# mit-han-lab/pvcnn

Hardware: AMD Instinct MI355X
Metric: point-clouds/sec fwd+bwd, PVCNN S3DIS N=4096 R=32 (higher is better)
Workload: dtype f32 (fp32 tensors, fp32 accumulate; Conv3d fwd / bwd-data / bwd-weight and the large SharedMLP fwd / bwd-data / bwd-weight products as power-of-two scaled fp16 hi+lo splits, 3 partial products on fp16 MFMA, max rel err vs fp64 1e-6 <= the fp32-MFMA kernels'; PVCNN_CONV_MATH=fp32 PVCNN_PW_MATH=fp32 s; 1 GPU; PVCNN (1xC) S3DIS fwd+bwd+Adam, B=16/GPU N=4096 R=32/16 fp32; global_batch=16, points=4096, parallelism=dp1, gradient_bytes=10289972, step_mode=graph, rccl_ranks=0, gradient_buckets=2

## Files before the change

include/pvcnn_hip.h:

```cpp
#ifndef PVCNN_HIP_H_
#define PVCNN_HIP_H_

#include <stddef.h>
#include <stdint.h>

#ifdef __cplusplus
extern "C" {
#endif

#if defined(__GNUC__)
#define PVCNN_API __attribute__((visibility("default")))
#else
#define PVCNN_API
#endif

#define PVCNN_ABI_VERSION 17
#define PVCNN_OK 0
#define PVCNN_ERR_INVALID_ARGUMENT (-1)

PVCNN_API int pvcnn_version(void);
PVCNN_API const char *pvcnn_last_error_string(void);

PVCNN_API int pvcnn_voxel_coords(const float *coords, int B, int N, int R, int normalize, float eps, float *norm_coords,
                       int32_t *vox_coords, void *stream);

PVCNN_API int pvcnn_voxel_coords_tail(const float *coords, long coords_batch_stride, const float *mean, const float *radius,
                            int B, int N, int R, float eps, float *norm_coords, int32_t *vox_coords, void *stream);

PVCNN_API size_t pvcnn_avg_voxelize_fwd_workspace_bytes(int B, int C, int N, int R);
PVCNN_API int pvcnn_avg_voxelize_fwd(const float *feat, const int32_t *coords, int B, int C, int N, int R,
                           float *out, int32_t *ind, int32_t *cnt, void *workspace,
                           size_t workspace_bytes, void *stream);
PVCNN_API int pvcnn_avg_voxelize_bwd(const float *grad_y, const int32_t *ind, const int32_t *cnt, int B,
                           int C, int N, int S, float *grad_x, void *stream);

PVCNN_API int pvcnn_trilinear_devox_fwd(const float *coords, const float *feat, int B, int C, int N, int R,
                              int is_training, int32_t *inds, float *wgts, float *outs,
                              void *stream);
PVCNN_API size_t pvcnn_trilinear_devox_bwd_workspace_bytes(int B, int C, int N, int R);
PVCNN_API int pvcnn_trilinear_devox_bwd(const float *grad_y, const int32_t *inds, const float *wgts, int B,
                              int C, int N, int R, float *grad_x, void *workspace,
                              size_t workspace_bytes, void *stream);

PVCNN_API size_t pvcnn_avg_voxelize_plan_bytes(int B, int N, int R);
PVCNN_API size_t pvcnn_avg_voxelize_plan_scratch_bytes(int B, int N, int R);
PVCNN_API int pvcnn_avg_voxelize_plan(const int32_t *coords, int B, int N, int R, int32_t *ind, int32_t *cnt, void *plan,
                            size_t plan_bytes, void *scratch, size_t scratch_bytes, void *stream);
PVCNN_API size_t pvcnn_pvconv_plans_scratch_bytes(int B, int N, int R);
PVCNN_API int pvcnn_pvconv_plans(const int32_t *vox_coords, const float *norm_coords, int B, int N, int R, int32_t *ind, int32_t *cnt,
                                 void *vox_plan, size_t vox_plan_bytes, void *devox_bwd_plan, size_t devox_bwd_plan_bytes,
                                 void *scratch, size_t scratch_bytes, void *stream);
PVCNN_API int pvcnn_avg_voxelize_apply(const float *feat, const void *plan, size_t plan_bytes, int B, int C, int N, int R,
                             float *out, void *stream);
PVCNN_API size_t pvcnn_trilinear_devox_bwd_plan_bytes(int B, int N, int R);
PVCNN_API size_t pvcnn_trilinear_devox_bwd_plan_scratch_bytes(int B, int N, int R);
PVCNN_API int pvcnn_trilinear_devox_bwd_plan(const int32_t *inds, const float *wgts, int B, int N, int R, void *plan,
                                   size_t plan_bytes, void *scratch, size_t scratch_bytes, void *stream);
PVCNN_API int pvcnn_trilinear_devox_bwd_apply(const float *grad_y, long grad_y_batch_stride, const void *plan, size_t plan_bytes,
                                    int B, int C, int N, int R, float *grad_x, void *stream);

PVCNN_API int pvcnn_ball_query(const float *centers, const float *points, int B, int N, int M, float radius,
                     int U, int32_t *out, void *stream);

PVCNN_API int pvcnn_grouping_fwd(const float *features, const int32_t *indices, int B, int C, int N, int M,
                       int U, float *out, void *stream);
PVCNN_API size_t pvcnn_grouping_bwd_workspace_bytes(int B, int C, int N, int M, int U);
PVCNN_API int pvcnn_grouping_bwd(const float *grad_y, const int32_t *indices, int B, int C, int N, int M,
// ... 387 lines not shown
```

pvcnn_amd/_lib.py:

```python
import ctypes
import functools
import os

import torch

_CSRC = os.path.join(os.path.dirname(os.path.abspath(__file__)), 'csrc')
LIB_PATH = os.path.join(_CSRC, 'libpvcnn_hip.so')
ABI_VERSION = 17

_vp, _i, _f, _sz, _l = ctypes.c_void_p, ctypes.c_int, ctypes.c_float, ctypes.c_size_t, ctypes.c_long
_ll = ctypes.c_longlong
_d = ctypes.c_double

SIGNATURES = {
    'pvcnn_version': (_i, []),
    'pvcnn_last_error_string': (ctypes.c_char_p, []),
    'pvcnn_voxel_coords': (_i, [_vp, _i, _i, _i, _i, _f, _vp, _vp, _vp]),
    'pvcnn_voxel_coords_tail': (_i, [_vp, ctypes.c_long, _vp, _vp, _i, _i, _i, _f, _vp, _vp, _vp]),
    'pvcnn_avg_voxelize_fwd_workspace_bytes': (_sz, [_i, _i, _i, _i]),
    'pvcnn_avg_voxelize_fwd': (_i, [_vp, _vp, _i, _i, _i, _i, _vp, _vp, _vp, _vp, _sz, _vp]),
    'pvcnn_avg_voxelize_bwd': (_i, [_vp, _vp, _vp, _i, _i, _i, _i, _vp, _vp]),
    'pvcnn_trilinear_devox_fwd': (_i, [_vp, _vp, _i, _i, _i, _i, _i, _vp, _vp, _vp, _vp]),
    'pvcnn_trilinear_devox_bwd_workspace_bytes': (_sz, [_i, _i, _i, _i]),
    'pvcnn_trilinear_devox_bwd': (_i, [_vp, _vp, _vp, _i, _i, _i, _i, _vp, _vp, _sz, _vp]),
    'pvcnn_avg_voxelize_plan_bytes': (_sz, [_i, _i, _i]),
    'pvcnn_avg_voxelize_plan_scratch_bytes': (_sz, [_i, _i, _i]),
    'pvcnn_avg_voxelize_plan': (_i, [_vp, _i, _i, _i, _vp, _vp, _vp, _sz, _vp, _sz, _vp]),
    'pvcnn_avg_voxelize_apply': (_i, [_vp, _vp, _sz, _i, _i, _i, _i, _vp, _vp]),
    'pvcnn_pvconv_plans_scratch_bytes': (_sz, [_i, _i, _i]),
    'pvcnn_pvconv_plans': (_i, [_vp, _vp, _i, _i, _i, _vp, _vp, _vp, _sz, _vp, _sz, _vp, _sz, _vp]),
    'pvcnn_trilinear_devox_bwd_plan_bytes': (_sz, [_i, _i, _i]),
    'pvcnn_trilinear_devox_bwd_plan_scratch_bytes': (_sz, [_i, _i, _i]),
    'pvcnn_trilinear_devox_bwd_plan': (_i, [_vp, _vp, _i, _i, _i, _vp, _sz, _vp, _sz, _vp]),
    'pvcnn_trilinear_devox_bwd_apply': (_i, [_vp, ctypes.c_long, _vp, _sz, _i, _i, _i, _i, _vp, _vp]),
    'pvcnn_ball_query': (_i, [_vp, _vp, _i, _i, _i, _f, _i, _vp, _vp]),
    'pvcnn_grouping_fwd': (_i, [_vp, _vp, _i, _i, _i, _i, _i, _vp, _vp]),
    'pvcnn_grouping_bwd_workspace_bytes': (_sz, [_i, _i, _i, _i, _i]),
    'pvcnn_grouping_bwd': (_i, [_vp, _vp, _i, _i, _i, _i, _i, _vp, _vp, _sz, _vp]),
    'pvcnn_gather_fwd': (_i, [_vp, _vp, _i, _i, _i, _i, _vp, _vp]),
    'pvcnn_gather_bwd_workspace_bytes': (_sz, [_i, _i, _i, _i]),
    'pvcnn_gather_bwd': (_i, [_vp, _vp, _i, _i, _i, _i, _vp, _vp, _sz, _vp]),
    'pvcnn_fps': (_i, [_vp, _i, _i, _i, _vp, _vp, _vp]),
    'pvcnn_mask_select': (_i, [_vp, _i, _i, _i, _vp, _vp, _vp, _vp, _vp]),
    'pvcnn_three_nn_interp_fwd': (_i, [_vp, _vp, _vp, _i, _i, _i, _i, _vp, _vp, _vp, _vp]),
    'pvcnn_three_nn_interp_bwd_workspace_bytes': (_sz, [_i, _i, _i, _i]),
    'pvcnn_three_nn_interp_bwd': (_i, [_vp, _vp, _vp, _i, _i, _i, _i, _vp, _vp, _sz, _vp]),
    'pvcnn_conv3d_weight_transform': (_i, [_vp, _i, _i, _i, _vp, _vp]),
    'pvcnn_conv3d_fwd': (_i, [_vp, _vp, _vp, _i, _i, _i, _i, _vp, _vp]),
    'pvcnn_conv3d_bwd_weight_workspace_bytes': (_sz, [_i, _i, _i, _i]),
    'pvcnn_conv3d_bwd_weight': (_i, [_vp, _vp, _i, _i, _i, _i, _vp, _vp, _vp, _sz, _vp]),
    'pvcnn_conv3d_weight_split_bytes': (_sz, [_i, _i, _i, _i]),
    'pvcnn_conv3d_weight_split': (_i, [_vp, _i, _i, _i, _i, _vp, _vp]),
    'pvcnn_conv3d_weight_split_pair': (_i, [_vp, _i, _i, _vp, _vp, _vp]),
    'pvcnn_conv3d_fwd_split_stats_parts': (_sz, [_i, _i, _i, _i]),
# ... 180 lines not shown
```

pvcnn_amd/csrc/slab.h:

```cpp
#pragma once
#include <algorithm>
#include <stdlib.h>

#include "common.h"

namespace pvcnn {

template <int NC>
struct Taps {
  int32_t idx[NC];
  float w[NC];
};

__device__ __forceinline__ float4 ld4(const float *p) { return *reinterpret_cast<const float4 *>(p); }
__device__ __forceinline__ int4 ld4(const int32_t *p) { return *reinterpret_cast<const int4 *>(p); }
__device__ __forceinline__ void st4(float *p, float a, float b, float c, float d) {
  *reinterpret_cast<float4 *>(p) = make_float4(a, b, c, d);
}
__device__ __forceinline__ void st4(int32_t *p, int a, int b, int c, int d) {
  *reinterpret_cast<int4 *>(p) = make_int4(a, b, c, d);
}

template <int NC, bool MAY_SKIP, bool PAD = false>
__device__ __forceinline__ float combine(const Taps<NC> &t, const float *row, int pshift = 0) {
// ... 191 lines not shown
};
struct XfBnAct {
  static constexpr bool kIdentity = false;
  static constexpr int kRaw = 5;
  const float *gamma, *beta, *mean, *rstd;
  float slope;
  const float *se = nullptr;
  __device__ __forceinline__ XfBnAct at(int b_times_C) const {
    XfBnAct x = *this;
    if (x.se) x.se += b_times_C;
    return x;
  }
  __device__ __forceinline__ void params(int c, float &scale, float &shift) const {
    scale = (gamma ? gamma[c] : 1.0f) * rstd[c];
    shift = (beta ? beta[c] : 0.0f) - mean[c] * scale;
  }
  __device__ __forceinline__ float mul(int c) const { return se ? se[c] : 1.0f; }
  __device__ __forceinline__ float apply(float v, float scale, float shift, float m = 1.0f) const {
    v = fmaf(v, scale, shift);
    v = v > 0.f ? v : v * slope;
    return se ? v * m : v;
  }
  __device__ __forceinline__ void fetch(int c, float (&raw)[5]) const {
    raw[0] = gamma ? gamma[c] : 1.0f; raw[1] = rstd[c]; raw[2] = beta ? beta[c] : 0.0f; raw[3] = mean[c]; raw[4] = mul(c);
  }
  __device__ __forceinline__ void combine(const float (&raw)[5], float &scale, float &shift) const {
    scale = raw[0] * raw[1];
    shift = raw[2] - raw[3] * scale;
  }
};

struct AddPlain {
  static constexpr bool kPlain = true;
};
struct AddBnAct {
  static constexpr bool kPlain = false;
  const float *gamma, *beta, *mean, *rstd;
  float slope;
  __device__ __forceinline__ void params(int c, float &scale, float &shift) const {
    scale = (gamma ? gamma[c] : 1.0f) * rstd[c];
    shift = (beta ? beta[c] : 0.0f) - mean[c] * scale;
  }
  __device__ __forceinline__ float apply(float a, float scale, float shift) const {
    const float v = fmaf(a, scale, shift);
    return v > 0.f ? v : v * slope;
  }
};

template <int THREADS, class XF>
__device__ __forceinline__ void slab_copy_row_xf(float *dst, const float *src, int len, const XF &xf, int c) {
  float scale, shift;
  xf.params(c, scale, shift);
  const float m = xf.mul(c);
  if (((reinterpret_cast<uintptr_t>(src) | reinterpret_cast<uintptr_t>(dst)) & 15) == 0 && (len & 3) == 0) {
    constexpr int kB = 8;
    const int nq = len >> 2;
    const float4 *s4 = reinterpret_cast<const float4 *>(src);
    float4 *d4 = reinterpret_cast<float4 *>(dst);
    for (int q0 = threadIdx.x; q0 < nq; q0 += THREADS * kB) {
      float4 v[kB];
#pragma unroll
      for (int u = 0; u < kB; ++u) v[u] = s4[min(q0 + u * THREADS, nq - 1)];
#pragma unroll
      for (int u = 0; u < kB; ++u)
        if (q0 + u * THREADS < nq)
          d4[q0 + u * THREADS] = make_float4(xf.apply(v[u].x, scale, shift, m), xf.apply(v[u].y, scale, shift, m),
                                             xf.apply(v[u].z, scale, shift, m), xf.apply(v[u].w, scale, shift, m));
    }
  } else {
    for (int i = threadIdx.x; i < len; i += THREADS) dst[i] = xf.apply(src[i], scale, shift, m);
  }
}

template <int THREADS, class XF>
__device__ __forceinline__ void slab_copy_row_padded(float *dst, const float *src, int len, int pshift, const XF &xf, int c) {
  float scale = 1.0f, shift = 0.0f;
  [[maybe_unused]] float m = 1.0f;
  if constexpr (!XF::kIdentity) { xf.params(c, scale, shift); m = xf.mul(c); }
  auto f = [&](float v) {
// ... 33 lines not shown

template <class P, int VEC, int THREADS, bool RESIDENT, class XF, bool PAD, class AX = AddPlain>
__global__ __launch_bounds__(THREADS) void gather_lds_kernel(P p, XF xf, const float *__restrict__ src,
                                                             float *__restrict__ dst, int C, int L,
                                                             int J, int G, int SEQ, int pshift,
                                                             const float *__restrict__ addend = nullptr, AX ax = AX{}) {
  extern __shared__ __attribute__((aligned(16))) float lds[];
  constexpr int NC = P::NC;
  const int b = blockIdx.y;
  const XF xfb = xf.at(b * C);
  const bool side = (blockIdx.x == 0);
  constexpr bool resident = RESIDENT;
  const int jf = threadIdx.x * VEC;
  typename P::Packed pk[VEC];
  if (resident && jf < J) {
    if constexpr (VEC == 4) p.pack4(b, jf, pk); else p.pack1(b, jf, pk[0]);
    if (side) {
      Taps<NC> t[VEC];
#pragma unroll
      for (int v = 0; v < VEC; ++v) p.unpack(pk[v], t[v]);
      if constexpr (VEC == 4) p.post4(b, jf, t); else p.post1(b, jf, t[0]);
    }
  }
  for (int sq = 0; sq < SEQ; ++sq) {
    const int c0 = (blockIdx.x * SEQ + sq) * G;
    if (c0 >= C) break;
    const int g = min(G, C - c0);
    if (sq > 0) lds_barrier();
    const int Lp = PAD ? L + (L >> pshift) : L;
    slab_stage<THREADS, PAD>(lds, src + ((size_t)b * C + c0) * L, g, L, Lp, pshift, xfb, c0);
    __syncthreads();
    float *out = dst + ((size_t)b * C + c0) * J;
    const float *add = addend ? addend + ((size_t)b * C + c0) * J : nullptr;
    for (int j0 = jf; j0 < J; j0 += THREADS * VEC) {
      Taps<NC> t[VEC];
      if constexpr (resident) {
#pragma unroll
        for (int v = 0; v < VEC; ++v) p.unpack(pk[v], t[v]);
      } else if constexpr (VEC == 4) {
        p.load4(b, j0, t);
        if (side && sq == 0) p.post4(b, j0, t);
      } else {
        p.load1(b, j0, t[0]);
        if (side && sq == 0) p.post1(b, j0, t[0]);
      }
      for (int c = 0; c < g; ++c) {
        const float *row = lds + c * Lp;
        [[maybe_unused]] float ascale = 1.0f, ashift = 0.0f;
        if constexpr (!AX::kPlain) ax.params(c0 + c, ascale, ashift);
        if constexpr (VEC == 4) {
          const float r0 = combine<NC, P::kMaySkip, PAD>(t[0], row, pshift), r1 = combine<NC, P::kMaySkip, PAD>(t[1], row, pshift);
          float r2 = combine<NC, P::kMaySkip, PAD>(t[2], row, pshift), r3 = combine<NC, P::kMaySkip, PAD>(t[3], row, pshift);
          float q0 = r0, q1 = r1;
          if (add) {
            float4 a = ld4(add + (size_t)c * J + j0);
            if constexpr (!AX::kPlain)
              a = make_float4(ax.apply(a.x, ascale, ashift), ax.apply(a.y, ascale, ashift), ax.apply(a.z, ascale, ashift), ax.apply(a.w, ascale, ashift));
            q0 = q0 + a.x; q1 = q1 + a.y; r2 = r2 + a.z; r3 = r3 + a.w;
          }
          st4(out + (size_t)c * J + j0, q0, q1, r2, r3);
        } else {
          float r = combine<NC, P::kMaySkip, PAD>(t[0], row, pshift);
          if (add) {
            float a = add[(size_t)c * J + j0];
            if constexpr (!AX::kPlain) a = ax.apply(a, ascale, ashift);
            r = r + a;
          }
          out[(size_t)c * J + j0] = r;
        }
      }
    }
  }
}

template <class P, class XF, class AX = AddPlain>
__global__ __launch_bounds__(1024) void gather_lds_pipe_kernel(P p, XF xf, const float *__restrict__ src, float *__restrict__ dst,
                                                               int C, int L, int J, int SEQ, int pshift,
                                                               const float *__restrict__ addend = nullptr, AX ax = AX{}) {
  extern __shared__ __attribute__((aligned(16))) float lds[];
  constexpr int NC = P::NC, THREADS = 1024, kB = 8;
  const int b = blockIdx.y;
  const XF xfb = xf.at(b * C);
  const int jf = threadIdx.x * 4;
  const bool has = jf < J;
  const int nq = L >> 2;
  float4 v[kB];
  typedef unsigned int u32x4 __attribute__((ext_vector_type(4)));
  const int voff = (int)threadIdx.x * 16;
  auto row_descriptor = [&](const float *base, size_t off, int bytes) {
    const uintptr_t rowp = reinterpret_cast<uintptr_t>(base + off);
    const uint32_t lo = __builtin_amdgcn_readfirstlane((uint32_t)rowp), hi = __builtin_amdgcn_readfirstlane((uint32_t)(rowp >> 32));
    return __builtin_amdgcn_make_buffer_rsrc(reinterpret_cast<void *>(((uintptr_t)hi << 32) | lo),  0,
                                              __builtin_amdgcn_readfirstlane(bytes), 0x00020000);
  };
  auto load = [&](const __amdgpu_buffer_rsrc_t &rsrc, int u) {
    const u32x4 raw = __builtin_amdgcn_raw_buffer_load_b128(rsrc, voff, u * THREADS * 16, 0);
// ... 268 lines not shown

template <class K>
inline int enable_big_lds(K kernel, size_t bytes) {
  if (bytes > 64 * 1024)
    return (int)hipFuncSetAttribute(reinterpret_cast<const void *>(kernel),
                                    hipFuncAttributeMaxDynamicSharedMemorySize, (int)bytes);
  return 0;
}

template <class P, class XF = XfNone, class AX = AddPlain>
int launch_gather(const P &p, const float *src, float *dst, int B, int C, int L, int J, bool vec_ok,
                  hipStream_t s, const char *what, const XF &xf = XF{}, int pshift = 0, const float *addend = nullptr,
                  const AX &ax = AX{}) {
  if (B == 0 || C == 0 || J == 0) return 0;
  if (!AX::kPlain && !addend) {
    set_error("%s: an addend transform needs an addend", what);
    return PVCNN_ERR_INVALID_ARGUMENT;
  }
  if (pshift > 0 && (size_t)(L + (L >> pshift)) * sizeof(float) > (size_t)kLdsBytesPerCU) pshift = 0;
  SlabPlan pl = plan_slab(B, C, L, pshift);
  if constexpr (P::kGridRows) {
    if (switches().gather_pipe && pl.lds && pshift > 0 && vec_ok && J <= 1024 * 4 && J > 1024 && (L >> 2) == 1024 && aligned16(src) && C >= 4) {
      constexpr int GR = 2;
      const int slabs = ceil_div(C, GR);
      const int seq = (int)std::min<long>(8, std::max<long>(1, (long)B * slabs / kNumCU));
      const size_t bytes = (size_t)GR * (L + (L >> pshift)) * sizeof(float);
      auto k = gather_lds_pipe_rows_kernel<P, XF, GR, AX>;
      if (int e = enable_big_lds(k, bytes)) { set_error("%s: LDS attribute: %d", what, e); return e; }
      hipLaunchKernelGGL(k, dim3(ceil_div(slabs, seq), B), dim3(1024), bytes, s, p, xf, src, dst, C, L, J, seq, pshift, addend, ax);
      return check_launch(what);
    }
  }
  if (!pl.lds) {
    if (!XF::kIdentity || addend || !AX::kPlain) {
      set_error("%s: row does not fit LDS; the fused transform / addend needs the LDS path", what);
      return PVCNN_ERR_INVALID_ARGUMENT;
    } else if constexpr (XF::kIdentity) {
      const int CT = 16;
      hipLaunchKernelGGL((gather_direct_kernel<P>), dim3(ceil_div(J, 256), ceil_div(C, CT), B), dim3(256), 0, s,
                         p, src, dst, C, L, J, CT);
      return check_launch(what);
    }
  }
  const dim3 grid(ceil_div(ceil_div(C, pl.G), pl.seq), B);
  if constexpr (P::kGridRows) {
    if (switches().gather_pipe && pl.threads == 1024 && pl.G == 1 && pshift > 0 && vec_ok && J <= 1024 * 4 && (L & 3) == 0 && (L >> 2) <= 1024 * 8 &&
        aligned16(src) && (((size_t)L * sizeof(float)) & 15) == 0) {
      auto k = gather_lds_pipe_kernel<P, XF, AX>;
      if (int e = enable_big_lds(k, pl.bytes)) { set_error("%s: LDS attribute: %d", what, e); return e; }
      hipLaunchKernelGGL(k, grid, dim3(1024), pl.bytes, s, p, xf, src, dst, C, L, J, pl.seq, pshift, addend, ax);
      return check_launch(what);
    }
  }
#define PVCNN_LAUNCH_GATHER_P(VEC, T, PADV)                                                      \
  do {                                                                                           \
    auto k = (J <= T * VEC) ? gather_lds_kernel<P, VEC, T, true, XF, PADV, AX> : gather_lds_kernel<P, VEC, T, false, XF, PADV, AX>; \
    if (int e = enable_big_lds(k, pl.bytes)) { set_error("%s: LDS attribute: %d", what, e); return e; } \
    hipLaunchKernelGGL(k, grid, dim3(T), pl.bytes, s, p, xf, src, dst, C, L, J, pl.G, pl.seq, pshift, addend, ax); \
  } while (0)
#define PVCNN_LAUNCH_GATHER(VEC, T)                                                              \
  do {                                                                                           \
    if constexpr (P::kGridRows) { if (pshift > 0) PVCNN_LAUNCH_GATHER_P(VEC, T, true); else PVCNN_LAUNCH_GATHER_P(VEC, T, false); } \
    else PVCNN_LAUNCH_GATHER_P(VEC, T, false);                                                   \
  } while (0)
  if (pl.threads == 1024) { if (vec_ok) PVCNN_LAUNCH_GATHER(4, 1024); else PVCNN_LAUNCH_GATHER(1, 1024); }
  else                    { if (vec_ok) PVCNN_LAUNCH_GATHER(4, 256);  else PVCNN_LAUNCH_GATHER(1, 256); }
#undef PVCNN_LAUNCH_GATHER
// ... 19 lines not shown
```

pvcnn_amd/csrc/voxelize.hip:

```cpp
#include <algorithm>

#include "csr.h"

namespace pvcnn {

__global__ __launch_bounds__(256) void vox_stats_atomic_kernel(const int32_t *__restrict__ coords, int N,
                                                               int R, int S, int32_t *__restrict__ ind,
                                                               int32_t *__restrict__ cnt) {
  const int b = blockIdx.y, i = blockIdx.x * 256 + threadIdx.x;
  if (i >= N) return;
  const int32_t *co = coords + (size_t)b * 3 * N;
  int v = co[i] * R * R + co[i + N] * R + co[i + 2 * N];
  v = min(max(v, 0), S - 1);
  ind[(size_t)b * N + i] = v;
  atomicAdd(cnt + (size_t)b * S + v, 1);
}

__global__ __launch_bounds__(256) void vox_scatter_atomic_kernel(
    const float *__restrict__ feat, const int32_t *__restrict__ ind, const int32_t *__restrict__ cnt, int C,
    int N, int S, int CT, float *__restrict__ out) {
  const int b = blockIdx.z, i = blockIdx.x * 256 + threadIdx.x;
  if (i >= N) return;
  const int pos = ind[(size_t)b * N + i];
  const int cur = cnt[(size_t)b * S + pos];
// ... 147 lines not shown
  if (!csr_supported(S, N)) {
    PVCNN_HIP_TRY(hipMemsetAsync(cnt, 0, (size_t)B * S * 4, s));
    PVCNN_HIP_TRY(hipMemsetAsync(out, 0, (size_t)B * C * S * 4, s));
    if (N == 0) return 0;
    hipLaunchKernelGGL(vox_stats_atomic_kernel, dim3(ceil_div(N, 256), B), dim3(256), 0, s, coords, N, R, S, ind, cnt);
    if (int e = check_launch("vox_stats_atomic")) return e;
    if (C == 0) return 0;
    const int CT = 16;
    hipLaunchKernelGGL(vox_scatter_atomic_kernel, dim3(ceil_div(N, 256), ceil_div(C, CT), B), dim3(256), 0, s,
                       feat, ind, cnt, C, N, S, CT, out);
    return check_launch("vox_scatter_atomic");
  }

  VoxelEntries ep{coords, ind, N, R, S};
  return launch_csr_scatter(ep, feat, out, B, C, S, N, N, cnt, workspace, workspace_bytes, s,
                            "avg_voxelize_fwd");
}

extern "C" int pvcnn_avg_voxelize_bwd(const float *grad_y, const int32_t *ind, const int32_t *cnt, int B, int C,
                                      int N, int S, float *grad_x, void *stream) {
  PVCNN_REQUIRE(B >= 0 && C >= 0 && N >= 0 && S > 0, "negative size");
  if (B == 0 || C == 0 || N == 0) return 0;
  PVCNN_REQUIRE(grad_y && ind && cnt && grad_x, "null pointer");
  PVCNN_REQUIRE(B <= 65535, "batch > 65535");
  VoxelMean p{ind, cnt, N, S};
  const bool vec = (N % 4 == 0) && aligned16(ind) && aligned16(grad_x);
  int pshift = 0;
  for (int k = 2; k <= 10; ++k)
    if ((1L << (3 * k)) == (long)S) pshift = k;
  return launch_gather(p, grad_y, grad_x, B, C, S, N, vec, static_cast<hipStream_t>(stream),
                       "avg_voxelize_bwd", XfNone{}, pshift);
}

extern "C" size_t pvcnn_avg_voxelize_plan_bytes(int B, int N, int R) {
  if (B <= 0 || N < 0 || R <= 0) return 0;
  const long S = (long)R * R * R;
  if (S > 0x7fffffffL / 4 || !csr_supported((int)S, N)) return 0;
  return CsrPlan::bytes(B, (int)S, N);
}

extern "C" size_t pvcnn_avg_voxelize_plan_scratch_bytes(int B, int N, int R) {
  if (B <= 0 || N < 0 || R <= 0) return 0;
  return csr_prep_scratch_bytes(B, N);
}

extern "C" int pvcnn_avg_voxelize_plan(const int32_t *coords, int B, int N, int R, int32_t *ind, int32_t *cnt, void *plan,
                                       size_t plan_bytes, void *scratch, size_t scratch_bytes, void *stream) {
  PVCNN_REQUIRE(B >= 0 && N >= 0 && R > 0, "negative size");
  PVCNN_REQUIRE((long)R * R * R <= 0x7fffffffL / 4, "resolution too large");
  const int S = R * R * R;
  if (B == 0) return 0;
  PVCNN_REQUIRE(csr_supported(S, N), "grid too large for a plan: use pvcnn_avg_voxelize_fwd");
  PVCNN_REQUIRE(cnt && (ind || N == 0) && (coords || N == 0), "null pointer");
  PVCNN_REQUIRE(B <= 65535, "batch > 65535");
  VoxelEntries ep{coords, ind, N, R, S};
  return launch_csr_prep(ep, B, S, N, cnt, plan, plan_bytes, scratch, scratch_bytes, static_cast<hipStream_t>(stream),
                         "avg_voxelize_plan");
}

extern "C" size_t pvcnn_pvconv_plans_scratch_bytes(int B, int N, int R) {
  if (B <= 0 || N < 0 || R <= 0) return 0;
  return csr_prep_scratch_bytes(B, N) + csr_prep_scratch_bytes(B, 8L * N);
}

extern "C" int pvcnn_pvconv_plans(const int32_t *vox_coords, const float *norm_coords, int B, int N, int R, int32_t *ind, int32_t *cnt,
                                  void *vox_plan, size_t vox_plan_bytes, void *devox_bwd_plan, size_t devox_bwd_plan_bytes, void *scratch,
// ... 51 lines not shown
```

pvcnn_amd/modules/functional/_product.py:

```python
from typing import Callable, NamedTuple

from . import _cache, _gradslots
from ._align import aligned as _aligned


class Product(NamedTuple):
    kind: str
    c: str
    canon: Callable
    canon_w: Callable
    shaped: Callable
    out_shape: Callable
    wgrad_shape: Callable
    bias_dims: tuple
    amax_seg: Callable
    amax_tiles: Callable
    stats_parts: Callable
    wgrad_f16_ok: Callable
    amax: str
    weight_images: str
    product_split: str

    def entry(self, lib, name):
        return getattr(lib, f'pvcnn_{self.c}_{name}')

    def method(self, be, name):
        return getattr(be, f'{self.c}_{name}')


def _same(t, shape=None):
    return t


CONV = Product(
    kind='conv', c='conv3d',
    canon=_same, canon_w=_same, shaped=_same,
    out_shape=lambda b, c, r: (b, c, r, r, r), wgrad_shape=lambda co, ci: (co, ci, 3, 3, 3), bias_dims=(0, 2, 3, 4),
    amax_seg=lambda be, r: r, amax_tiles=lambda b, r, seg: b * r * r,
    stats_parts=lambda b, c, r, nsplit: (b, c, r, nsplit),
    wgrad_f16_ok=lambda be, x, w: True,
    amax='conv_amax', weight_images='conv_weight_images', product_split='conv3d_igemm_split')

PW = Product(
    kind='pw', c='pwconv',
    canon=lambda t: t.view(t.shape[0], t.shape[1], -1), canon_w=lambda w: w.view(w.shape[0], w.shape[1]),
    shaped=lambda t, shape: t.view(shape),
    out_shape=lambda b, c, n: (b, c, n), wgrad_shape=lambda co, ci: (co, ci), bias_dims=(0, 2),
    amax_seg=lambda be, n: be.PW_AMAX_SEG, amax_tiles=lambda b, n, seg: b * ((n + seg - 1) // seg),
    stats_parts=lambda b, c, n, nsplit: (b, n),
    wgrad_f16_ok=lambda be, x, w: x.shape[0] * x.shape[2] * w.shape[0] * w.shape[1] >= getattr(be, 'pw_wgrad_f16_min_macs', 0),
    amax='pw_amax', weight_images='pw_weight_images', product_split='pwconv_gemm_split')


def forward(p, be, ctx, given, weight, bias, want_stats, nsplit):
    x, w = p.canon(_aligned(given)), p.canon_w(weight.contiguous())
    ctx.save_for_backward(x, w)
    ctx.has_bias, ctx.x_shape, ctx.w_shape = bias is not None, given.shape, weight.shape
    ctx.bias_param = bias
    ctx.nsplit = int(nsplit)
    b = bias.contiguous() if bias is not None else None
    ctx.x_amax = None
    if ctx.nsplit in (1, 2):
        ctx.x_amax = _cache.amax_of(given, p.amax_seg(be, x.shape[2]))
        if ctx.x_amax is None and ctx.nsplit == 2:
            ctx.x_amax = getattr(be, p.amax)(x, want_global=False)
    kw = {'amax': ctx.x_amax} if ctx.nsplit == 2 else {}
    ctx.w_bwd_image = None
    if ctx.nsplit and hasattr(be, p.weight_images) and ctx.needs_input_grad[0]:
        w_image, ctx.w_bwd_image = getattr(be, p.weight_images)(w, ctx.nsplit)
        run = lambda **k: getattr(be, p.product_split)(x, w_image, b, w.shape[0], ctx.nsplit, amax=ctx.x_amax, **k)
    elif ctx.nsplit:
        run = lambda **k: p.method(be, 'forward_split')(x, w, b, ctx.nsplit, **kw, **k)
    else:
        run = lambda **k: p.method(be, 'forward')(x, w, b, **k)
    y_shape = (given.shape[0], w.shape[0], *given.shape[2:])
    if want_stats:
        y, part = run(want_stats=True)
        ctx.mark_non_differentiable(part)
        ctx.set_materialize_grads(False)
        return p.shaped(y, y_shape), part
    return p.shaped(run(), y_shape)


def backward(p, be, ctx, received):
    x, w = ctx.saved_tensors
    if received is None:
        return None, None, None, None, None
    grad_y = p.canon(_aligned(received))
    f16 = ctx.nsplit == 2
    wgrad_f16 = (ctx.nsplit in (1, 2) and ctx.needs_input_grad[1] and p.method(be, 'backward_weight_f16_serves')(x)
                 and p.wgrad_f16_ok(be, x, w))
    g_amax = None
    if (f16 and (ctx.needs_input_grad[0] or wgrad_f16)) or (ctx.nsplit == 1 and wgrad_f16):
        g_amax = _cache.amax_of(received, p.amax_seg(be, grad_y.shape[2]))
        if g_amax is None and f16:
            g_amax = getattr(be, p.amax)(grad_y, want_global=False)
    gx = None
    if ctx.needs_input_grad[0]:
        if ctx.nsplit and ctx.w_bwd_image is not None:
            rows = getattr(ctx, 'need_rows', None)
            gx = getattr(be, p.product_split)(grad_y, ctx.w_bwd_image, None, w.shape[1], ctx.nsplit, False, g_amax,
                                              **({'rows': rows} if rows is not None else {}))
        elif ctx.nsplit:
            gx = p.method(be, 'backward_data_split')(grad_y, w, ctx.nsplit, **({'amax': g_amax} if f16 else {}))
        else:
            gx = p.method(be, 'backward_data')(grad_y, w)
        gx = p.shaped(gx, ctx.x_shape)
    want_bias = ctx.has_bias and ctx.needs_input_grad[2]
    gw = gb = None
    if ctx.needs_input_grad[1]:
        dst = _gradslots.destinations(be, w, ctx.bias_param if want_bias else None)
        res = (p.method(be, 'backward_weight_f16')(x, grad_y, ctx.x_amax, g_amax, with_bias=want_bias, **dst) if wgrad_f16
               else p.method(be, 'backward_weight')(x, grad_y, with_bias=want_bias, **dst))
        gw, gb = res if want_bias else (res, None)
        gw = p.shaped(gw, ctx.w_shape)
    elif want_bias:
        gb = grad_y.sum(dim=p.bias_dims)
    return gx, gw, gb, None, None
```

pvcnn_amd/modules/functional/backend.py:

```python
import ctypes
import os

import torch

from ... import _lib
from . import _cache
from ._align import aligned as _aligned
from ._product import CONV, PW

__all__ = ['_backend']


def _dev(t, name):
    if not t.is_cuda:
        raise RuntimeError(f'{name} must be a CUDA (HIP) tensor -- the PVConv hot path has no CPU implementation')


def _f32(t, name):
    _dev(t, name)
    if not t.is_contiguous():
        raise RuntimeError(f'{name} must be a contiguous tensor')
    if t.dtype != torch.float32:
        raise RuntimeError(f'{name} must be a float tensor')

# ... 335 lines not shown
               'avg_voxelize: features (B,C,N), coords (B,3,N) expected')
        b, c, n = features.shape
        r = int(resolution)
        s3 = r * r * r
        dev = features.device
        if self.seam_plan_memo and self.lib.pvcnn_avg_voxelize_plan_bytes(b, n, r):
            key = ('seam voxelize plan', r)
            hit = _cache.memo(coords, key, lambda: self._stamped_voxel_plan(coords, r))
            if hit is not None and (hit[0].ind._version, hit[0].cnt._version) != hit[1]:
                _cache.forget(coords, key)
                hit = _cache.memo(coords, key, lambda: self._stamped_voxel_plan(coords, r))
            if hit is not None:
                return [self.avg_voxelize_apply(features, hit[0]), hit[0].ind, hit[0].cnt]
        out = torch.empty((b, c, s3), dtype=torch.float32, device=dev)
        ind = torch.empty((b, n), dtype=torch.int32, device=dev)
        cnt = torch.empty((b, s3), dtype=torch.int32, device=dev)
        ws = self._scratch(self.lib.pvcnn_avg_voxelize_fwd_workspace_bytes(b, c, n, r), dev)
        _run(self.lib.pvcnn_avg_voxelize_fwd, 'avg_voxelize_forward', features, features, coords, b, c, n, r, out, ind, cnt, ws, ws.numel())
        return [out, ind, cnt]

    def _stamped_voxel_plan(self, coords, r):
        vp = self.avg_voxelize_plan(coords, r)
        return None if vp is None else (vp, (vp.ind._version, vp.cnt._version))

    def avg_voxelize_backward(self, grad_y, indices, cnt):
        _f32(grad_y, 'grad_y'); _i32(indices, 'indices'); _i32(cnt, 'cnt')
        _shape(grad_y.dim() == 3 and indices.dim() == 2 and tuple(cnt.shape) == (grad_y.shape[0], grad_y.shape[2])
               and indices.shape[0] == grad_y.shape[0],
               'avg_voxelize backward: grad_y (B,C,S), indices (B,N), cnt (B,S) expected')
        b, c, s3 = grad_y.shape
        n = indices.shape[1]
        grad_x = torch.empty((b, c, n), dtype=torch.float32, device=grad_y.device)
        _run(self.lib.pvcnn_avg_voxelize_bwd, 'avg_voxelize_backward', grad_y, grad_y, indices, cnt, b, c, n, s3, grad_x)
        return grad_x

    has_scatter_plans = True

    class VoxelPlan:
        __slots__ = ('ind', 'cnt', 'plan', 'r', 'n', 'b')

    def _voxel_plan(self, b, n, r, nbytes, dev):
        vp = self.VoxelPlan()
        vp.r, vp.n, vp.b = r, n, b
        vp.ind = torch.empty((b, n), dtype=torch.int32, device=dev)
        vp.cnt = torch.empty((b, r * r * r), dtype=torch.int32, device=dev)
        vp.plan = torch.empty((nbytes,), dtype=torch.uint8, device=dev)
        return vp

    def avg_voxelize_plan(self, coords, resolution):
        _i32(coords, 'coords')
        _shape(coords.dim() == 3 and coords.shape[1] == 3, 'avg_voxelize: coords (B,3,N) expected')
        b, _, n = coords.shape
        r = int(resolution)
        nbytes = self.lib.pvcnn_avg_voxelize_plan_bytes(b, n, r)
        if nbytes == 0:
            return None
        vp = self._voxel_plan(b, n, r, nbytes, coords.device)
        scratch = self._scratch(self.lib.pvcnn_avg_voxelize_plan_scratch_bytes(b, n, r), coords.device)
        _run(self.lib.pvcnn_avg_voxelize_plan, 'avg_voxelize_plan', coords, coords, b, n, r, vp.ind, vp.cnt, vp.plan, vp.plan.numel(),
             scratch, scratch.numel())
        return vp

    has_conv_bwd_rows = True

    def voxel_need_rows(self, cnt, resolution):
        _i32(cnt, 'cnt')
# ... 1121 lines not shown
```

pvcnn_amd/modules/functional/voxelization.py:

```python
from torch.autograd import Function

from . import _cache
from ._autograd import native, amp_fwd, amp_bwd

__all__ = ['avg_voxelize']


class AvgVoxelization(Function):

    @staticmethod
    @amp_fwd
    def forward(ctx, features, coords, resolution):
        r = int(resolution)
        feats = features.contiguous()
        be = native()
        plan = None
        if feats.is_cuda and getattr(be, 'has_scatter_plans', False):
            plan = _cache.memo(coords, ('avg_voxelize_plan', r), lambda: be.avg_voxelize_plan(coords.int().contiguous(), r))
        if plan is not None:
            grid, point_voxel, voxel_count = be.avg_voxelize_apply(feats, plan), plan.ind, plan.cnt
        else:
            grid, point_voxel, voxel_count = be.avg_voxelize_forward(feats, coords.int().contiguous(), r)
        ctx.save_for_backward(point_voxel, voxel_count)
        return grid.view(feats.shape[0], feats.shape[1], r, r, r)

    @staticmethod
    @amp_bwd
    def backward(ctx, grad_grid):
        point_voxel, voxel_count = ctx.saved_tensors
        nb, nc = grad_grid.shape[0], grad_grid.shape[1]
        flat = grad_grid.contiguous().view(nb, nc, -1)
        return native().avg_voxelize_backward(flat, point_voxel, voxel_count), None, None


avg_voxelize = AvgVoxelization.apply
```

pvcnn_amd/modules/pvconv.py:

```python
import torch
import torch.nn as nn

from . import functional as F
from .functional._autograd import native
from .functional.bnact import (batch_norm_act_devoxelize, batch_norm_act_devoxelize_point_bn, batch_norm_act_se_devoxelize, fusable_tail,
                               point_bn_fusable, run_layers, _has_hooks)
from .functional.conv3d import conv_nsplit, voxel_conv3d
from .se import SE3d
from .shared_mlp import SharedMLP
from .voxelization import Voxelization

__all__ = ['PVConv']


class _VoxelConv3d(nn.Conv3d):

    def _fast(self, x):
        return (x.is_cuda and getattr(native(), 'has_conv3d', False) and self.kernel_size == (3, 3, 3)
                and self.stride == (1, 1, 1) and self.padding == (1, 1, 1) and self.dilation == (1, 1, 1)
                and self.groups == 1 and self.padding_mode == 'zeros' and x.dim() == 5
                and x.shape[2] == x.shape[3] == x.shape[4] and self.weight.dtype == torch.float32
                and (x.dtype == torch.float32 or (torch.is_autocast_enabled() and x.dtype in (torch.bfloat16, torch.float16))))

    def forward(self, x):
        if not self._fast(x):
            return super().forward(x)
        return voxel_conv3d(x, self.weight, self.bias, False, conv_nsplit())

    def forward_with_stats(self, x, need_rows=None):
        if not self._fast(x):
            return self.forward(x)
        return voxel_conv3d(x, self.weight, self.bias, True, conv_nsplit(), need_rows)


class PVConv(nn.Module):
    def __init__(self, in_channels, out_channels, kernel_size, resolution, with_se=False, normalize=True, eps=0):
# ... 4 lines not shown
        self.resolution = resolution

        self.voxelization = Voxelization(resolution, normalize=normalize, eps=eps)
        pad = kernel_size // 2
        grid_ops = []
        for cin in (in_channels, out_channels):
            grid_ops += [_VoxelConv3d(cin, out_channels, kernel_size, stride=1, padding=pad),
                         nn.BatchNorm3d(out_channels, eps=1e-4),
                         nn.LeakyReLU(0.1, True)]
        if with_se:
            grid_ops.append(SE3d(out_channels))
        self.voxel_layers = nn.Sequential(*grid_ops)
        self.point_features = SharedMLP(in_channels, out_channels)

    def _point_branch_in_gather(self, features, bn, se):
        if se is not None or not (self.training and bn.training) or not isinstance(self.point_features, SharedMLP):
            return None
        if _has_hooks(self.point_features):
            return None
        found = point_bn_fusable(self.point_features.layers, features, self.training)
        return None if found is None else found[1:]

    def _need_rows(self, grid, coords):
        if not (self.training and torch.is_grad_enabled() and grid.is_cuda and grid.requires_grad and len(self.voxel_layers) > 1):
            return None
        conv, bn = self.voxel_layers[0], self.voxel_layers[1]
        if not (isinstance(conv, _VoxelConv3d) and conv._fast(grid) and conv_nsplit() != 0
                and isinstance(bn, nn.modules.batchnorm._BatchNorm) and bn.training):
            return None
        if any(_has_hooks(m) for m in (self, self.voxelization, self.voxel_layers, *self.voxel_layers)):
            return None
        return self.voxelization.needed_rows(coords)

    def forward(self, inputs):
        features, coords = inputs
        grid, grid_coords = self.voxelization(features, coords)
        need_rows = self._need_rows(grid, coords)
        tail = fusable_tail(self.voxel_layers, grid) if self.resolution ** 3 * 4 <= 160 * 1024 else None
        if tail is not None:
            bn, slope, se = tail
            ntail = 2 if se is None else 3
            grid, stats_part = run_layers(self.voxel_layers, grid, stop=len(self.voxel_layers) - ntail, tail_stats=True,
                                          first_need_rows=need_rows)
            point = self._point_branch_in_gather(features, bn, se)
            if point is not None:
                p_bn, p_slope = point
                pre, p_stats = run_layers(self.point_features.layers, features, stop=1, tail_stats=True)
                return batch_norm_act_devoxelize_point_bn(grid, grid_coords, bn, slope, self.resolution, stats_part,
                                                          pre, p_bn, p_slope, p_stats), coords
            per_point = self.point_features(features)
            if se is None:
                fused = batch_norm_act_devoxelize(grid, grid_coords, bn, slope, self.resolution, self.training, stats_part,
                                                  addend=per_point)
            else:
                fused = batch_norm_act_se_devoxelize(grid, grid_coords, bn, slope, se, self.resolution, self.training, stats_part,
                                                     addend=per_point)
            return fused, coords
        else:
            hooked = bool(self.voxel_layers._forward_hooks or self.voxel_layers._forward_pre_hooks or self.voxel_layers._backward_hooks)
            grid = self.voxel_layers(grid) if hooked else run_layers(self.voxel_layers, grid, first_need_rows=need_rows)
            per_point = self.point_features(features)
            from_voxels = F.trilinear_devoxelize(grid, grid_coords, self.resolution, self.training)
        return from_voxels + per_point, coords
```

pvcnn_amd/workload.py:

```python
import contextlib

import torch
import torch.nn as nn

from .modules import PVConv, PointNetAModule, PointNetFPModule, PointNetSAModule, SharedMLP
from .modules.functional.bnact import emit_row_max, run_layers
from .modules.functional.dense import run_dense

SEED = 1588147245

__all__ = ['PVCNN', 'PVCNN2', 'PVCNNShapeNet', 'FrustumPVCNNE', 'make_s3dis_batch', 'make_shapenet_batch',
           'make_frustum_batch', 'make_frustum_targets', 'frustum_size_templates', 'SEED']


def _scaled(width, k):
    return int(k * width)


class _TapAndPool(torch.autograd.Function):

    @staticmethod
    def forward(ctx, x, winners, values=None):
        ctx.save_for_backward(winners)
        ctx.npoints = x.shape[-1]
        return x.view_as(x), (values.view_as(values) if values is not None else x.gather(2, winners.unsqueeze(-1)).squeeze(-1))

    @staticmethod
    def backward(ctx, g_tap, g_pool):
        (winners,) = ctx.saved_tensors
        if g_tap is None and g_pool is None:
            return None, None, None
        if g_tap is None:
            g = torch.zeros(g_pool.shape + (int(ctx.npoints),), dtype=g_pool.dtype, device=g_pool.device)
        elif getattr(g_tap, '_pvcnn_private_slice', False) and not torch.is_grad_enabled():
            g = g_tap
        else:
            g = g_tap.clone(memory_format=torch.contiguous_format)
        if g_pool is not None:
            g.scatter_add_(2, winners.unsqueeze(-1), g_pool.unsqueeze(-1).to(g.dtype))
        return g, None, None


class _ConcatPoints(torch.autograd.Function):

    @staticmethod
    def forward(ctx, spec, *taps):
        from .modules.functional._autograd import native
        be = native()
        ctx.splits = [t.shape[1] for t in taps]
        if spec is None:
            out, amax = be.concat_points([t.detach() for t in taps], want_global=False)
        else:
            out, amax = be.concat_points([t.detach() for t in taps], out=spec[0], in_place=spec[1], want_global=False)
        ctx.mark_non_differentiable(amax)
        ctx.set_materialize_grads(False)
        return out, amax

    @staticmethod
    def backward(ctx, grad, _grad_amax=None):
        if grad is None:
            return (None,) * (1 + len(ctx.splits))
        grads, off = [None], 0
        for c in ctx.splits:
            piece = grad.narrow(1, off, c)
            piece._pvcnn_private_slice = True
            grads.append(piece)
            off += c
        return tuple(grads)


_SLOT_ENABLED = __import__('os').environ.get('PVCNN_CONCAT_SLOT', '1') != '0'


class _Slot:

    def __init__(self, buffer, index, c0, c1):
        self.buffer, self.index, self.view = buffer, index, buffer[:, c0:c1, :]

    def holds(self, tap):
        v = self.view
        return (tap.data_ptr() == v.data_ptr() and tuple(tap.shape) == tuple(v.shape) and tuple(tap.stride()) == tuple(v.stride()))


def concat_slot(taps_so_far, stage_channels, total_channels, like, training=True):
    from .modules.functional._autograd import native
    if not (_SLOT_ENABLED and training and like.is_cuda and like.dtype == torch.float32 and torch.is_grad_enabled()):
        return None
    be = native()
    if not (getattr(be, 'has_concat_points', False) and getattr(be, 'has_bnact_rowmax', False)) or like.shape[-1] % 256:
        return None
    if getattr(be, 'pw_math', '') != 'f16x2':
        return None
    c0 = sum(int(t.shape[1]) for t in taps_so_far)
    if c0 + stage_channels > total_channels:
        return None
    buf = torch.empty((like.shape[0], int(total_channels), like.shape[-1]), dtype=torch.float32, device=like.device)
    return _Slot(buf, len(taps_so_far), c0, c0 + int(stage_channels))


# ... 491 lines not shown
```

Measured before the change: 2596 point-clouds/s.

## Fuse PVConv input gradient accumulation into avg-voxelize backward gather

Adds a gradient-join mechanism. The point-branch SharedMLP backward-data gradient and the concat slice gradient for a PVConv input are deposited instead of being returned to autograd. The avg-voxelize backward kernel then adds up to two addends while writing grad_x, which removes the separate elementwise accumulation kernels and the extra read/write passes autograd would otherwise emit. The cost is fragile autograd-engine bookkeeping (pass ids, callbacks, will-execute checks) that raises an error if a deposited gradient is never collected.

```diff
diff --git a/include/pvcnn_hip.h b/include/pvcnn_hip.h
--- a/include/pvcnn_hip.h
+++ b/include/pvcnn_hip.h
@@ -33,6 +33,9 @@
                            size_t workspace_bytes, void *stream);
 PVCNN_API int pvcnn_avg_voxelize_bwd(const float *grad_y, const int32_t *ind, const int32_t *cnt, int B,
                            int C, int N, int S, float *grad_x, void *stream);
+PVCNN_API int pvcnn_avg_voxelize_bwd_add(const float *grad_y, const int32_t *ind, const int32_t *cnt, int B, int C, int N,
+                               int S, const float *add0, long add0_batch_stride, const float *add1,
+                               long add1_batch_stride, float *grad_x, void *stream);
 
 PVCNN_API int pvcnn_trilinear_devox_fwd(const float *coords, const float *feat, int B, int C, int N, int R,
                               int is_training, int32_t *inds, float *wgts, float *outs,
diff --git a/pvcnn_amd/_lib.py b/pvcnn_amd/_lib.py
--- a/pvcnn_amd/_lib.py
+++ b/pvcnn_amd/_lib.py
@@ -20,6 +20,7 @@
     'pvcnn_avg_voxelize_fwd_workspace_bytes': (_sz, [_i, _i, _i, _i]),
     'pvcnn_avg_voxelize_fwd': (_i, [_vp, _vp, _i, _i, _i, _i, _vp, _vp, _vp, _vp, _sz, _vp]),
     'pvcnn_avg_voxelize_bwd': (_i, [_vp, _vp, _vp, _i, _i, _i, _i, _vp, _vp]),
+    'pvcnn_avg_voxelize_bwd_add': (_i, [_vp, _vp, _vp, _i, _i, _i, _i, _vp, _l, _vp, _l, _vp, _vp]),
     'pvcnn_trilinear_devox_fwd': (_i, [_vp, _vp, _i, _i, _i, _i, _i, _vp, _vp, _vp, _vp]),
     'pvcnn_trilinear_devox_bwd_workspace_bytes': (_sz, [_i, _i, _i, _i]),
     'pvcnn_trilinear_devox_bwd': (_i, [_vp, _vp, _vp, _i, _i, _i, _i, _vp, _vp, _sz, _vp]),
diff --git a/pvcnn_amd/csrc/slab.h b/pvcnn_amd/csrc/slab.h
--- a/pvcnn_amd/csrc/slab.h
+++ b/pvcnn_amd/csrc/slab.h
@@ -247,9 +247,11 @@
 
 struct AddPlain {
   static constexpr bool kPlain = true;
+  static constexpr bool kJoin = false;
 };
 struct AddBnAct {
   static constexpr bool kPlain = false;
+  static constexpr bool kJoin = false;
   const float *gamma, *beta, *mean, *rstd;
   float slope;
   __device__ __forceinline__ void params(int c, float &scale, float &shift) const {
@@ -260,6 +262,13 @@
     const float v = fmaf(a, scale, shift);
     return v > 0.f ? v : v * slope;
   }
+};
+
+struct AddJoin {
+  static constexpr bool kPlain = true;
+  static constexpr bool kJoin = true;
+  const float *a0, *a1;
+  long s0, s1;
 };
 
 template <int THREADS, class XF>
@@ -359,6 +368,11 @@
     __syncthreads();
     float *out = dst + ((size_t)b * C + c0) * J;
     const float *add = addend ? addend + ((size_t)b * C + c0) * J : nullptr;
+    [[maybe_unused]] const float *ja0 = nullptr, *ja1 = nullptr;
+    if constexpr (AX::kJoin) {
+      ja0 = ax.a0 + (size_t)b * ax.s0 + (size_t)c0 * J;
+      if (ax.a1) ja1 = ax.a1 + (size_t)b * ax.s1 + (size_t)c0 * J;
+    }
     for (int j0 = jf; j0 < J; j0 += THREADS * VEC) {
       Taps<NC> t[VEC];
       if constexpr (resident) {
@@ -379,7 +393,14 @@
           const float r0 = combine<NC, P::kMaySkip, PAD>(t[0], row, pshift), r1 = combine<NC, P::kMaySkip, PAD>(t[1], row, pshift);
           float r2 = combine<NC, P::kMaySkip, PAD>(t[2], row, pshift), r3 = combine<NC, P::kMaySkip, PAD>(t[3], row, pshift);
           float q0 = r0, q1 = r1;
-          if (add) {
+          if constexpr (AX::kJoin) {
+            float4 a = ld4(ja0 + (size_t)c * J + j0);
+            if (ja1) {
+              const float4 e = ld4(ja1 + (size_t)c * J + j0);
+              a = make_float4(a.x + e.x, a.y + e.y, a.z + e.z, a.w + e.w);
+            }
+            q0 = a.x + q0; q1 = a.y + q1; r2 = a.z + r2; r3 = a.w + r3;
+          } else if (add) {
             float4 a = ld4(add + (size_t)c * J + j0);
             if constexpr (!AX::kPlain)
               a = make_float4(ax.apply(a.x, ascale, ashift), ax.apply(a.y, ascale, ashift), ax.apply(a.z, ascale, ashift), ax.apply(a.w, ascale, ashift));
@@ -388,7 +409,11 @@
           st4(out + (size_t)c * J + j0, q0, q1, r2, r3);
         } else {
           float r = combine<NC, P::kMaySkip, PAD>(t[0], row, pshift);
-          if (add) {
+          if constexpr (AX::kJoin) {
+            float a = ja0[(size_t)c * J + j0];
+            if (ja1) a = a + ja1[(size_t)c * J + j0];
+            r = a + r;
+          } else if (add) {
             float a = add[(size_t)c * J + j0];
             if constexpr (!AX::kPlain) a = ax.apply(a, ascale, ashift);
             r = r + a;
@@ -723,7 +748,7 @@
     }
   }
   if (!pl.lds) {
-    if (!XF::kIdentity || addend || !AX::kPlain) {
+    if (!XF::kIdentity || addend || !AX::kPlain || AX::kJoin) {
       set_error("%s: row does not fit LDS; the fused transform / addend needs the LDS path", what);
       return PVCNN_ERR_INVALID_ARGUMENT;
     } else if constexpr (XF::kIdentity) {
diff --git a/pvcnn_amd/csrc/voxelize.hip b/pvcnn_amd/csrc/voxelize.hip
--- a/pvcnn_amd/csrc/voxelize.hip
+++ b/pvcnn_amd/csrc/voxelize.hip
@@ -203,6 +203,28 @@
                        "avg_voxelize_bwd", XfNone{}, pshift);
 }
 
+extern "C" int pvcnn_avg_voxelize_bwd_add(const float *grad_y, const int32_t *ind, const int32_t *cnt, int B, int C, int N, int S,
+                                          const float *add0, long add0_batch_stride, const float *add1, long add1_batch_stride,
+                                          float *grad_x, void *stream) {
+  if (!add0) { add0 = add1; add0_batch_stride = add1_batch_stride; add1 = nullptr; }
+  if (!add0) return pvcnn_avg_voxelize_bwd(grad_y, ind, cnt, B, C, N, S, grad_x, stream);
+  PVCNN_REQUIRE(B >= 0 && C >= 0 && N >= 0 && S > 0, "negative size");
+  if (B == 0 || C == 0 || N == 0) return 0;
+  PVCNN_REQUIRE(grad_y && ind && cnt && grad_x, "null pointer");
+  PVCNN_REQUIRE(B <= 65535, "batch > 65535");
+  PVCNN_REQUIRE(add0_batch_stride >= (long)C * N && (!add1 || add1_batch_stride >= (long)C * N), "addend batch stride smaller than one cloud");
+  PVCNN_REQUIRE(add0 != grad_x && add1 != grad_x, "an addend may not be the output");
+  AddJoin ax{add0, add1, add0_batch_stride, add1 ? add1_batch_stride : 0L};
+  VoxelMean p{ind, cnt, N, S};
+  const bool vec = (N % 4 == 0) && aligned16(ind) && aligned16(grad_x) && aligned16(add0) && add0_batch_stride % 4 == 0 &&
+                   (!add1 || (aligned16(add1) && add1_batch_stride % 4 == 0));
+  int pshift = 0;
+  for (int k = 2; k <= 10; ++k)
+    if ((1L << (3 * k)) == (long)S) pshift = k;
+  return launch_gather(p, grad_y, grad_x, B, C, S, N, vec, static_cast<hipStream_t>(stream), "avg_voxelize_bwd_add", XfNone{},
+                       pshift, nullptr, ax);
+}
+
 extern "C" size_t pvcnn_avg_voxelize_plan_bytes(int B, int N, int R) {
   if (B <= 0 || N < 0 || R <= 0) return 0;
   const long S = (long)R * R * R;
diff --git a/pvcnn_amd/modules/functional/_gradjoin.py b/pvcnn_amd/modules/functional/_gradjoin.py
--- /dev/null
+++ b/pvcnn_amd/modules/functional/_gradjoin.py
@@ -0,0 +1,83 @@
+import os
+import weakref
+
+import torch
+from torch.autograd import Variable
+
+enabled = os.environ.get('PVCNN_GRAD_JOIN', '1') != '0'
+
+_ATTR = '_pvcnn_grad_join'
+
+
+def _pass_id():
+    fn = getattr(torch._C, '_current_graph_task_id', None)
+    return fn() if fn is not None else -1
+
+
+class GradJoin:
+
+    def __init__(self, name, capacity=2, accepts=None):
+        self.name, self.capacity, self.accepts = str(name), int(capacity), accepts
+        self.armed = False
+        self.spent = False
+        self._held = []
+        self._pass = None
+        self._closer = None
+
+    def arm(self, node=None):
+        self.armed = True
+        self._closer = weakref.ref(node) if node is not None else None
+        return self
+
+    def _closer_runs(self):
+        if self._closer is None:
+            return True
+        node, ask = self._closer(), getattr(torch._C, '_will_engine_execute_node', None)
+        if node is None:
+            return False
+        try:
+            return True if ask is None else bool(ask(node))
+        except RuntimeError:
+            return True
+
+    def deposit(self, grad):
+        if grad is None or not enabled or not self.armed or self.spent or torch.is_grad_enabled():
+            return False
+        now = _pass_id()
+        if self._held and self._pass != now:
+            self._held = []
+            self.spent = True
+            return False
+        if len(self._held) >= self.capacity or (self.accepts is not None and not self.accepts(grad)) or not self._closer_runs():
+            return False
+        if not self._held:
+            self._pass = now
+            Variable._execution_engine.queue_callback(self._end_of_pass)
+        self._held.append(grad)
+        return True
+
+    def collect(self):
+        held, self._held = self._held, []
+        if held and self._pass != _pass_id():
+            held = []
+        self.spent = True
+        return held
+
+    def _end_of_pass(self):
+        if self._held:
+            n, self._held, self.spent = len(self._held), [], True
+            raise RuntimeError(f'gradient join of {self.name}: {n} deposited gradient(s) were never collected -- the closing reader '
+                               f'of the tensor did not run in this backward pass, so the gradient would be incomplete '
+                               f'(PVCNN_GRAD_JOIN=0 turns the join off)')
+
+
+def open(tensor, name, capacity=2, accepts=None):
+    if not (enabled and torch.is_grad_enabled() and tensor.requires_grad):
+        return None
+    join = GradJoin(name, capacity, accepts)
+    setattr(tensor, _ATTR, join)
+    return join
+
+
+def of(tensor):
+    return getattr(tensor, _ATTR, None) if enabled else None
diff --git a/pvcnn_amd/modules/functional/_product.py b/pvcnn_amd/modules/functional/_product.py
--- a/pvcnn_amd/modules/functional/_product.py
+++ b/pvcnn_amd/modules/functional/_product.py
@@ -1,6 +1,6 @@
 from typing import Callable, NamedTuple
 
-from . import _cache, _gradslots
+from . import _cache, _gradjoin, _gradslots
 from ._align import aligned as _aligned
 
 
@@ -58,6 +58,7 @@
     ctx.has_bias, ctx.x_shape, ctx.w_shape = bias is not None, given.shape, weight.shape
     ctx.bias_param = bias
     ctx.nsplit = int(nsplit)
+    ctx.grad_join = _gradjoin.of(given) if ctx.needs_input_grad[0] else None
     b = bias.contiguous() if bias is not None else None
     ctx.x_amax = None
     if ctx.nsplit in (1, 2):
@@ -106,6 +107,8 @@
         else:
             gx = p.method(be, 'backward_data')(grad_y, w)
         gx = p.shaped(gx, ctx.x_shape)
+        if ctx.grad_join is not None and ctx.grad_join.deposit(gx):
+            gx = None
     want_bias = ctx.has_bias and ctx.needs_input_grad[2]
     gw = gb = None
     if ctx.needs_input_grad[1]:
diff --git a/pvcnn_amd/modules/functional/backend.py b/pvcnn_amd/modules/functional/backend.py
--- a/pvcnn_amd/modules/functional/backend.py
+++ b/pvcnn_amd/modules/functional/backend.py
@@ -391,6 +391,25 @@
         n = indices.shape[1]
         grad_x = torch.empty((b, c, n), dtype=torch.float32, device=grad_y.device)
         _run(self.lib.pvcnn_avg_voxelize_bwd, 'avg_voxelize_backward', grad_y, grad_y, indices, cnt, b, c, n, s3, grad_x)
+        return grad_x
+
+    has_grad_join = True
+
+    def avg_voxelize_backward_add(self, grad_y, indices, cnt, addends):
+        if not addends:
+            return self.avg_voxelize_backward(grad_y, indices, cnt)
+        _f32(grad_y, 'grad_y'); _i32(indices, 'indices'); _i32(cnt, 'cnt')
+        _arg(grad_y.dim() == 3 and indices.dim() == 2, 'avg_voxelize backward: grad_y (B,C,S), indices (B,N) expected')
+        b, c, s3 = grad_y.shape
+        n = indices.shape[1]
+        _arg(len(addends) <= 2 and tuple(cnt.shape) == (b, s3) and tuple(indices.shape) == (b, n)
+               and all(tuple(a.shape) == (b, c, n) and a.device == grad_y.device for a in addends),
+               'avg_voxelize backward: grad_y (B,C,S), indices (B,N), cnt (B,S) and at most two (B,C,N) addends expected')
+        strides = [_f32_rows(a, 'addend') for a in addends]
+        a0, a1 = addends[0], (addends[1] if len(addends) > 1 else None)
+        grad_x = torch.empty((b, c, n), dtype=torch.float32, device=grad_y.device)
+        _run(self.lib.pvcnn_avg_voxelize_bwd_add, 'avg_voxelize_backward_add', grad_y, grad_y, indices, cnt, b, c, n, s3,
+             a0, strides[0], a1, strides[1] if a1 is not None else 0, grad_x)
         return grad_x
 
     has_scatter_plans = True
diff --git a/pvcnn_amd/modules/functional/voxelization.py b/pvcnn_amd/modules/functional/voxelization.py
--- a/pvcnn_amd/modules/functional/voxelization.py
+++ b/pvcnn_amd/modules/functional/voxelization.py
@@ -1,6 +1,6 @@
 from torch.autograd import Function
 
-from . import _cache
+from . import _cache, _gradjoin
 from ._autograd import native, amp_fwd, amp_bwd
 
 __all__ = ['avg_voxelize']
@@ -22,6 +22,8 @@
         else:
             grid, point_voxel, voxel_count = be.avg_voxelize_forward(feats, coords.int().contiguous(), r)
         ctx.save_for_backward(point_voxel, voxel_count)
+        join = _gradjoin.of(features)
+        ctx.grad_join = join.arm(ctx) if (join is not None and ctx.needs_input_grad[0] and getattr(be, 'has_grad_join', False)) else None
         return grid.view(feats.shape[0], feats.shape[1], r, r, r)
 
     @staticmethod
@@ -30,6 +32,9 @@
         point_voxel, voxel_count = ctx.saved_tensors
         nb, nc = grad_grid.shape[0], grad_grid.shape[1]
         flat = grad_grid.contiguous().view(nb, nc, -1)
+        earlier = ctx.grad_join.collect() if ctx.grad_join is not None else []
+        if earlier:
+            return native().avg_voxelize_backward_add(flat, point_voxel, voxel_count, earlier), None, None
         return native().avg_voxelize_backward(flat, point_voxel, voxel_count), None, None
 
 
diff --git a/pvcnn_amd/modules/pvconv.py b/pvcnn_amd/modules/pvconv.py
--- a/pvcnn_amd/modules/pvconv.py
+++ b/pvcnn_amd/modules/pvconv.py
@@ -2,6 +2,7 @@
 import torch.nn as nn
 
 from . import functional as F
+from .functional import _gradjoin
 from .functional._autograd import native
 from .functional.bnact import (batch_norm_act_devoxelize, batch_norm_act_devoxelize_point_bn, batch_norm_act_se_devoxelize, fusable_tail,
                                point_bn_fusable, run_layers, _has_hooks)
@@ -72,8 +73,22 @@
             return None
         return self.voxelization.needed_rows(coords)
 
+    def _join_input_gradients(self, features):
+        if not (_gradjoin.enabled and torch.is_tensor(features) and features.is_cuda and features.dtype == torch.float32
+                and features.dim() == 3 and features.requires_grad and torch.is_grad_enabled() and not torch.is_autocast_enabled()
+                and getattr(native(), 'has_grad_join', False) and isinstance(self.point_features, SharedMLP)):
+            return None
+        point = self.point_features
+        if any(_has_hooks(m) for m in (self, self.voxelization, point, point.layers, *point.layers)):
+            return None
+        from .functional.backend import batch_strided_ok
+        shape, device = tuple(features.shape), features.device
+        return _gradjoin.open(features, f'PVConv({self.in_channels}, {self.out_channels}, R={self.resolution}) input {shape}', capacity=2,
+                              accepts=lambda g: tuple(g.shape) == shape and g.device == device and batch_strided_ok(g))
+
     def forward(self, inputs):
         features, coords = inputs
+        self._join_input_gradients(features)
         grid, grid_coords = self.voxelization(features, coords)
         need_rows = self._need_rows(grid, coords)
         tail = fusable_tail(self.voxel_layers, grid) if self.resolution ** 3 * 4 <= 160 * 1024 else None
diff --git a/pvcnn_amd/workload.py b/pvcnn_amd/workload.py
--- a/pvcnn_amd/workload.py
+++ b/pvcnn_amd/workload.py
@@ -4,6 +4,7 @@
 import torch.nn as nn
 
 from .modules import PVConv, PointNetAModule, PointNetFPModule, PointNetSAModule, SharedMLP
+from .modules.functional import _gradjoin
 from .modules.functional.bnact import emit_row_max, run_layers
 from .modules.functional.dense import run_dense
 
@@ -48,6 +49,7 @@
         from .modules.functional._autograd import native
         be = native()
         ctx.splits = [t.shape[1] for t in taps]
+        ctx.joins = [_gradjoin.of(t) if ctx.needs_input_grad[1 + i] else None for i, t in enumerate(taps)]
         if spec is None:
             out, amax = be.concat_points([t.detach() for t in taps], want_global=False)
         else:
@@ -61,10 +63,10 @@
         if grad is None:
             return (None,) * (1 + len(ctx.splits))
         grads, off = [None], 0
-        for c in ctx.splits:
+        for c, join in zip(ctx.splits, ctx.joins):
             piece = grad.narrow(1, off, c)
             piece._pvcnn_private_slice = True
-            grads.append(piece)
+            grads.append(None if (join is not None and join.deposit(piece)) else piece)
             off += c
         return tuple(grads)
 
```

New measurement: 2617 point-clouds/s (median of 6 runs). Within noise of the previous version (+0.8%).
